# tgale96/sputnik

Hardware: AMD Instinct MI355X
Metric: effective TFLOP/s (nnz-FLOPs) DSD block=128 M=K=N=4096 @ 1/2/4/8 GPU vs density (higher is better)
Workload: dtype f16

## Files before the change

### sputnik_amd/csrc/api_internal.h

```cpp
#ifndef SPUTNIK_AMD_API_INTERNAL_H_
#define SPUTNIK_AMD_API_INTERNAL_H_

#include <cstddef>

#include "sputnik/block/arguments.h"

namespace sputnik_amd {

enum class Status {
  kOk,
  kNotSupported,
  kNoKernel,
  kMissingMetadata,
  kMissingRowIndices,
};

using sputnik::block::BlockMatrix;
using sputnik::block::Matrix;

struct Workspace {
  void *ptr = nullptr;
  size_t bytes = 0;
};

// ... 76 lines not shown
void SetPairFault(int on);
int CaptureWorkspaces();
int SelectDsdKernel(int four_wave);
bool Dsd4wEnabled();
bool Dsd4wForced();
int Dsd4wEpi();

enum KnobId {
  kKnobPairs,
  kKnobPairXcd2,
  kKnobSplit,
  kKnobSplitMinBn,
  kKnobDsd4w,
  kKnobGroupedSdd,
  kKnobGroupedMinPerCu,
  kKnobTall,
  kKnobTallPersistent,
  kKnobDdsXcd2,
  kKnobSdd4wMaxLd,
  kKnobPairFault,
  kKnobSddKsplit,
  kKnobSddKsplitMinK,
  kKnobSddOrder,
  kKnobTall4w,
  kKnobTallFlushW,
  kKnobTallOddShare,
  kKnobMinHandoff,
  kKnobXcdRows,
  kKnobSddKrot,
  kKnobSddSpread,
  kKnobSddBtMinMib,
  kKnobSddTailMinK,
  kKnobSddActRoute,
  kNumKnobs
};
int Knob(KnobId k);
int TuningGet(const char *name);
int TuningSet(const char *name, int value);

}

#endif
```

### sputnik_amd/csrc/block_gemm.h

```cpp
#ifndef SPUTNIK_AMD_BLOCK_GEMM_H_
#define SPUTNIK_AMD_BLOCK_GEMM_H_

#include <hip/hip_runtime.h>
#include <stdint.h>

#include <type_traits>

#include "act_math.h"

#ifndef SPUTNIK_EXP
#define SPUTNIK_EXP 0
#endif
#ifndef SPUTNIK_S_AUX
#define SPUTNIK_S_AUX 0
#endif
#ifndef SPUTNIK_D_AUX
#define SPUTNIK_D_AUX 0
#endif
#ifndef SPUTNIK_IDX_PREFETCH
#define SPUTNIK_IDX_PREFETCH 0
#endif
#ifndef SPUTNIK_READ_FIRST
#define SPUTNIK_READ_FIRST 0
#endif
// ... 56 lines not shown
  int grid;
  int persistent;
  unsigned long long *tile_counter;
  int pair;
  float *pair_partials;
  unsigned *pair_flags;
  unsigned pair_epoch;
  unsigned *pair_sync;
  unsigned *pair_error;
  int pair_fault;
  int pair_xcd2;
  int pair_split;
  int split_bn;
  unsigned long long *debug;
  const int *d_offsets;
  const short *d_indices;
  const int *d_block_offsets;
  int s_blocks;
  int sdd_ksplit;
  unsigned *ks_flags;
  int sdd_order;
  int tall_flush_w;
  int tall_odd_share;
  int min_handoff;
  int xcd_rows;
  int sdd_krot;
  int sdd_spread;
  int sdd_tail;
  int tail_cus;
  char *z_data;
  int act;
  char *u_data;
  char *du_data;
};

__device__ __forceinline__ int tr_key(int k) {
  return (k & 3) | (((k >> 3) & 1) << 2);
}
template <int kChunks>
__device__ __forceinline__ int kc_key(int row) {
  return (row >> 1) & (kChunks - 1);
}

template <typename T>
struct MfmaTraits;
template <>
struct MfmaTraits<_Float16> {
  static __device__ __forceinline__ f32x4 mfma(s16x8 a, s16x8 b, f32x4 c) {
    return __builtin_amdgcn_mfma_f32_16x16x32_f16(
        __builtin_bit_cast(f16x8, a), __builtin_bit_cast(f16x8, b), c, 0, 0,
        0);
  }
};
template <>
struct MfmaTraits<__bf16> {
  static __device__ __forceinline__ f32x4 mfma(s16x8 a, s16x8 b, f32x4 c) {
    return __builtin_amdgcn_mfma_f32_16x16x32_bf16(
        __builtin_bit_cast(bf16x8, a), __builtin_bit_cast(bf16x8, b), c, 0, 0,
        0);
  }
};

template <int N>
__device__ __forceinline__ void wait_vmcnt() {
  asm volatile("s_waitcnt vmcnt(%0)" ::"n"(N) : "memory");
}
// ... 1618 lines not shown
```

### sputnik_amd/csrc/dispatch.cpp

```cpp
#include <atomic>
#include <cstdint>
#include <cstdlib>
#include <cstring>
#include <mutex>

#include "api_internal.h"
#include "block_gemm.h"
#include "dsd4w.h"
#include "layout.h"
#include "metadata.h"
#include "sputnik/sputnik.h"
#include "sputnik_amd.h"

namespace sputnik_amd {

static unsigned long long *g_debug = nullptr;

constexpr int kMaxDevices = 64;

static std::atomic<unsigned long long> g_incall_events{0};
static std::atomic<unsigned long long> g_bt_launches{0};
static thread_local int t_product_depth = 0;
struct InProduct {
  InProduct() { ++t_product_depth; }
// ... 37 lines not shown
static std::mutex g_pairs_mu;

struct KnobDef {
  const char *name;
  const char *env;
  int def, lo, hi;
};
static const KnobDef kKnobs[kNumKnobs] = {
    {"pairs", "SPUTNIK_AMD_PAIRS", 1, 0, 1},
    {"pair_xcd2", "SPUTNIK_AMD_PAIR_XCD2", 3, 0, 3},
    {"split", "SPUTNIK_AMD_SPLIT", 1, 0, 1},
    {"split_min_bn", "SPUTNIK_AMD_SPLIT_MIN_BN", 128, 0, 1 << 20},
    {"dsd4w", "SPUTNIK_AMD_DSD4W", 1, 0, 7},
    {"grouped_sdd", "SPUTNIK_AMD_GROUPED_SDD", 1, 0, 1},
    {"grouped_min_per_cu", "SPUTNIK_AMD_GROUPED_MIN_PER_CU", 4, 0, 1 << 20},
    {"tall", "SPUTNIK_AMD_TALL", 1, 0, 2},
    {"tall_persistent", "SPUTNIK_AMD_TALL_PERSISTENT", 1, 0, 1},
    {"dds_xcd2", "SPUTNIK_AMD_DDS_XCD2", 3, 0, 3},
    {"sdd4w_max_ld", "SPUTNIK_AMD_SDD4W_MAX_LD", 16384, 0, 1 << 30},
    {"pair_fault", "SPUTNIK_AMD_PAIR_FAULT", 0, 0, 1},
    {"sdd_ksplit", "SPUTNIK_AMD_SDD_KSPLIT", 1, 1, 8},
    {"sdd_ksplit_min_k", "SPUTNIK_AMD_SDD_KSPLIT_MIN_K", 6144, 512, 1 << 30},
    {"sdd_order", "SPUTNIK_AMD_SDD_ORDER", 1, 0, 4},
    {"tall4w", "SPUTNIK_AMD_TALL4W", 1, 0, 1},
    {"tall_flush_w", "SPUTNIK_AMD_TALL_FLUSH_W", 4, 0, 64},
    {"tall_odd_share", "SPUTNIK_AMD_TALL_ODD_SHARE", 120, 50, 200},
    {"min_handoff", "SPUTNIK_AMD_MIN_HANDOFF", 2, 1, 64},
    {"xcd_rows", "SPUTNIK_AMD_XCD_ROWS", 1, 0, 1},
    {"sdd_krot", "SPUTNIK_AMD_SDD_KROT", 0, 0, 4},
    {"sdd_spread", "SPUTNIK_AMD_SDD_SPREAD", 2, 0, 2},
    {"sdd_bt_min_mib", "SPUTNIK_AMD_SDD_BT_MIN_MIB", 256, 0, 1 << 20},
    {"sdd_tail_min_k", "SPUTNIK_AMD_SDD_TAIL_MIN_K", 8192, 0, 1 << 30},
    {"sdd_act_route", "SPUTNIK_AMD_SDD_ACT_ROUTE", 0, 0, 2},
};
constexpr int kKnobUnset = -0x7fffffff - 1;
static std::atomic<int> g_knobs[kNumKnobs];
static std::once_flag g_knobs_once;

static void InitKnobs() {
  std::call_once(g_knobs_once, [] {
    for (int i = 0; i < kNumKnobs; ++i) {
      const char *e = std::getenv(kKnobs[i].env);
      char *end = nullptr;
      const long v0 = e != nullptr && *e != 0 ? std::strtol(e, &end, 10) : 0;
      const bool ok = e != nullptr && *e != 0 && end != nullptr && *end == 0 &&
                      v0 >= kKnobs[i].lo && v0 <= kKnobs[i].hi;
      const int v = ok ? (int)v0 : kKnobs[i].def;
      g_knobs[i].store(v, std::memory_order_relaxed);
    }
  });
}

int Knob(KnobId k) {
  InitKnobs();
  return g_knobs[k].load(std::memory_order_relaxed);
}

static int KnobIndex(const char *name) {
  if (name == nullptr) return -1;
  for (int i = 0; i < kNumKnobs; ++i)
    if (std::strcmp(name, kKnobs[i].name) == 0) return i;
  return -1;
}

int TuningGet(const char *name) {
  const int i = KnobIndex(name);
// ... 1021 lines not shown
        return RunDsd(a, ta, Matrix(b.cols, b.rows, bt), false, c, dtype, build_meta, stream,
                      st_out, Workspace{}, OutMode::kStore);
      }
    }
  }
  if (needs_meta && build_meta) {
    const hipError_t e = BuildTransposed(a, stream);
    if (e != hipSuccess) return e;
  }
  p.debug = g_debug;
  p.xcd_rows = Knob(kKnobXcdRows);
  PreparePairs(&p, a.nonzeros / (kBlock * kBlock), stream);
  const GemmParams p0 = p;
  GemmParams pd = p;
  const bool tall = UseTall(&pd, stream, true);
  if (tall && UseTallPipe(p0, a.nonzeros / (kBlock * kBlock),
                          ((long long)a.cols + kBlock - 1) / kBlock, ta, tb)) {
    GemmParams q = p0;
    q.persistent = 0;
    q.num_jtiles = q.j_limit / 512;
    q.tall_flush_w = Knob(kKnobTallFlushW);
    q.tall_odd_share = Knob(kKnobTallOddShare);
    int dev = 0;
    q.num_tiles = hipGetDevice(&dev) == hipSuccess ? DeviceCUs(dev) : 0;
    return LaunchDsd4w(dtype, q, 7, false, stream, false, false);
  }
  if (tall) (void)UseTall(&p, stream);
  if (Dsd4wEnabled() &&
      Dsd4wApplies(p, Dsd4wForced() ? (1LL << 40) : a.nonzeros / (kBlock * kBlock),
                   !ta, tb, false, tall)) {
    int epi = Dsd4wEpi();
    if (Dsd4wMode() == 1 && a.nonzeros / (kBlock * kBlock) < 12LL * p.num_rows)
      epi = 5;
    return LaunchDsd4w(dtype, p, epi, tb && !ta, stream, ta && !tb, ta && tb);
  }
  return LaunchBlockGemm(dtype, false, !ta, tb, false, tall, p, stream);
}

hipError_t RunDds(const Matrix &a, bool ta, const BlockMatrix &b, bool tb,
                  const Matrix &c, int dtype, bool build_meta,
                  hipStream_t stream, Status *st_out, OutMode out) {
  const InProduct in_product;
  GemmParams p;
  bool needs_meta = false;
  const Status st = PrepareDds(a, ta, b, tb, c, &p, &needs_meta);
  *st_out = st;
  if (st != Status::kOk) return hipSuccess;
  if (needs_meta && build_meta) {
    const hipError_t e = BuildTransposed(b, stream);
    if (e != hipSuccess) return e;
  }
  p.debug = g_debug;
  if (out != OutMode::kStore) {
    if (out == OutMode::kAccF32) p.c_ld *= 2;
    PreparePairs(&p, b.nonzeros / (kBlock * kBlock), stream, false,
                 false);
    const bool tall = UseTall(&p, stream);
    return LaunchBlockGemmAcc(dtype, tb, !ta,
                              true, tall,
                              out == OutMode::kAccF32 ? kOutAccF32 : kOutAccT,
                              p, stream);
  }
  p.xcd_rows = Knob(kKnobXcdRows);
  PreparePairs(&p, b.nonzeros / (kBlock * kBlock), stream);
  const bool tall = UseTall(&p, stream);
  if (Dsd4wEnabled() &&
// ... 707 lines not shown
```

### sputnik_amd/csrc/dsd4w.hip

```cpp
#include <hip/hip_runtime.h>
#include <stdint.h>

#include <cstdlib>

#include "api_internal.h"
#include "block_gemm.h"
#include "dsd4w.h"
#include "dsd4w_asm.inc"

namespace sputnik_amd {
namespace {

constexpr int kRankScratch = 24576;
constexpr uint32_t kOob = 0x80000000u;

struct Pick {
  int row_a, row_b, e_a, n_a, e_b, n_b, target;
  int uniform;
};

__device__ Pick rank_wave(const GemmParams &p, char *lds, int wave, int lane,
                          int ra, int rb, int o0_pre, bool pre) {
  const int R = p.num_rows;
  const int o0 = pre ? o0_pre : lane <= R ? p.s_offsets[lane] : 0;
// ... 78 lines not shown
  out.n_b = __builtin_amdgcn_readfirstlane(offs[out.row_b + 1]) - out.e_b;
  __syncthreads();
  return out;
}

__device__ __forceinline__ unsigned long long exp_stamp(int dep) {
#if (SPUTNIK_EXP & 512) != 0
  unsigned long long t;
  asm volatile("s_memrealtime %0\n s_waitcnt lgkmcnt(0)"
               : "=s"(t) : "s"(__builtin_amdgcn_readfirstlane(dep)));
  return t;
#else
  (void)dep;
  return 0;
#endif
}

template <bool kBf16, int kEpi, bool kDds, bool kSdd = false, bool kNt = false,
          bool kTt = false, bool kTn = false>
__global__ void __launch_bounds__(256, 1) dsd4w_kernel(const GemmParams p) {
  constexpr bool kWaveEpi = kEpi != 0;
  constexpr bool kDs = kEpi == 3 || kEpi == 4 || kEpi == 5 || kEpi == 6 || kEpi == 7;
  constexpr bool kBar2 = kEpi == 4;
  constexpr bool kKs = kEpi == 6;
  constexpr bool kTp = kEpi == 7;
  static_assert(!kTp || (!kSdd && !kDds && !kNt && !kTt && !kTn), "tall pipeline: DSD NN");
  static_assert(!kDds || kEpi == 1 || kEpi == 3, "DDS: per-wave epilogue only");
  static_assert(!kSdd || ((kEpi == 3 || (kEpi == 4 && !kTt) || (kEpi == 1 && kTn) ||
                           (kKs && !kNt && !kTt && !kTn)) && !kDds),
                "SDD: double slots (TN: per-step images), per-wave epilogue");
  static_assert(!kKs || kSdd, "K-split: SDD NN only");
  constexpr bool kARowsT = (kTt || kTn) && kSdd;
  constexpr bool kDdsTt = kDds && kTt;
  [[maybe_unused]] const unsigned long long t_entry = __builtin_amdgcn_s_memrealtime();
  __shared__ __attribute__((aligned(1024))) char lds[163840];
  const int tid = threadIdx.x;
  const int lane = tid & 63;
  const int wave = __builtin_amdgcn_readfirstlane(tid >> 6);
  const uint32_t lbase =
      (uint32_t)(uintptr_t)((__attribute__((address_space(3))) char *)lds);

  constexpr int kIdxPreload = 1024;
  const int nb_all = p.s_blocks;
  [[maybe_unused]] const unsigned long long t_karg = exp_stamp(nb_all);
  const bool idx_pre = nb_all <= kIdxPreload &&
                       (reinterpret_cast<uintptr_t>(p.s_indices) & 15) == 0;
  typedef unsigned v4u_t __attribute__((ext_vector_type(4)));
  v4u_t idx_lo = {0u, 0u, 0u, 0u}, idx_hi = {0u, 0u, 0u, 0u};
  if (idx_pre) {
    const __amdgpu_buffer_rsrc_t ri = __builtin_amdgcn_make_buffer_rsrc(
        const_cast<short *>(p.s_indices), 0, (nb_all * 2 + 3) & ~3, 0x00020000);
    idx_lo = __builtin_bit_cast(v4u_t, __builtin_amdgcn_raw_buffer_load_b128(
                                            ri, lane * 32, 0, 0));
    idx_hi = __builtin_bit_cast(v4u_t, __builtin_amdgcn_raw_buffer_load_b128(
                                            ri, lane * 32 + 16, 0, 0));
  }
#ifndef SPUTNIK_OFF_EARLY
#define SPUTNIK_OFF_EARLY 1
#endif
  const bool off_early = SPUTNIK_OFF_EARLY && !kSdd && !kTp && p.num_rows < 64;
  int off_pre = 0;
  if (off_early && lane <= p.num_rows) off_pre = p.s_offsets[lane];
  auto kblock_of = [&](int e) {
    if constexpr (kSdd) return e;
    if (!idx_pre || e >= nb_all) return scalar_load_short(p.s_indices, e);
    const int l = e >> 4, d = (e & 15) >> 1;
    const unsigned w0 = __builtin_amdgcn_readlane(idx_lo.x, l);
    const unsigned w1 = __builtin_amdgcn_readlane(idx_lo.y, l);
    const unsigned w2 = __builtin_amdgcn_readlane(idx_lo.z, l);
    const unsigned w3 = __builtin_amdgcn_readlane(idx_lo.w, l);
    const unsigned w4 = __builtin_amdgcn_readlane(idx_hi.x, l);
    const unsigned w5 = __builtin_amdgcn_readlane(idx_hi.y, l);
    const unsigned w6 = __builtin_amdgcn_readlane(idx_hi.z, l);
    const unsigned w7 = __builtin_amdgcn_readlane(idx_hi.w, l);
    const unsigned w = d == 0 ? w0 : d == 1 ? w1 : d == 2 ? w2 : d == 3 ? w3
                     : d == 4 ? w4 : d == 5 ? w5 : d == 6 ? w6 : w7;
    return (int)((e & 1) ? (w >> 16) : (w & 0xffff));
  };

  int srow, j0;
  int b1, n1, b2 = 0, n2 = 0;
  bool producer = false, collect = false;
  int pair_id = 0;
  [[maybe_unused]] unsigned long long t_rank = 0;
  unsigned epoch = p.pair_epoch;
  if (p.pair != 0 && p.pair_sync != nullptr)
    epoch = ((unsigned)scalar_load_int(reinterpret_cast<const int *>(p.pair_sync), 0) &
             0x7fffffffu) + 1u;
  int grp_b0 = 0, grp_count = 0, grp_c = 0;
  bool split_idle = false;
  int kss = 1, kch = 0, kofs = 0;
  unsigned tp_ent = 0, tp_tile = 0, tp_ent2 = 0, tp_tile2 = 0, tp_zero = 0xffffffffu;
  int tp_first = 0, tp_second = 0, tp_nzero = 0;
  if constexpr (kSdd) {
    int tile = xcd_tile(blockIdx.x, gridDim.x);
    const int R = !kKs && p.sdd_tail != 0
                      ? sdd_tail_rows<256>(p, reinterpret_cast<int *>(lds + kRankScratch), tid)
                      : p.num_rows;
    const bool band = p.sdd_order >= 1;
    const int per = band ? ((R + 255) / 256 + 7) & ~7 : (R + 255) / 256;
    const int r0 = min(R, tid * per), r1 = min(R, r0 + per);
    int local = 0, gmin = 0x7fffffff, gmax = 0;
    for (int r = r0; r < r1; ++r) {
      const int gr = (p.c_offsets[r + 1] - p.c_offsets[r] + 3) / 4;
      local += gr;
      gmin = min(gmin, gr);
      gmax = max(gmax, gr);
    }
    int incl = local;
#pragma unroll
    for (int d = 1; d < 64; d <<= 1) {
      const int v = __shfl_up(incl, d, 64);
      if (lane >= d) incl += v;
    }
#pragma unroll
    for (int d = 1; d < 64; d <<= 1) {
      gmin = min(gmin, __shfl_xor(gmin, d, 64));
      gmax = max(gmax, __shfl_xor(gmax, d, 64));
    }
    int *wsum = reinterpret_cast<int *>(lds + kRankScratch);
    if (lane == 63) {
      wsum[wave] = incl;
      wsum[4 + wave] = gmin;
      wsum[8 + wave] = gmax;
// ... 224 lines not shown
      }
      __syncthreads();
      tp_nzero = min(64, zhi - zlo);
      tp_zero = lane < tp_nzero ? (unsigned)zl[lane] : 0xffffffffu;
    }
    __syncthreads();
    j0 = 0;
    srow = 0;
    b1 = 0;
    n1 = nblk;
    tp_first = (int)(__builtin_amdgcn_readlane(tp_ent, 0) & 0xffffffu);
    tp_second = (int)(__builtin_amdgcn_readlane(tp_ent, nblk > 1 ? 1 : 0) & 0xffffffu);
    split_idle = nblk == 0;
  } else if (p.pair != 0 && p.pair_split == 2) {
    const int nt = p.num_tiles;
    const int gch = (int)blockIdx.x >= nt ? 1 : 0;
    const int t = xcd_tile((int)blockIdx.x - gch * nt, nt);
    srow = t % p.num_rows;
    j0 = (t / p.num_rows) * 512;
    const int e_r = scalar_load_int(p.s_offsets, srow);
    const int n_r = scalar_load_int(p.s_offsets, srow + 1) - e_r;
    const int c0 = gch * n_r / 2, c1 = (gch + 1) * n_r / 2;
    b1 = e_r + c0;
    n1 = c1 - c0;
    pair_id = t;
    if (gch == 0) {
      producer = n1 > 0;
      split_idle = n1 == 0;
    } else {
      collect = n_r / 2 > 0;
    }
  } else if (p.pair != 0) {
    const int R = p.num_rows;
    const int half = R >> 1;
    const int n_light = p.num_jtiles * half;
    const int n_solo = p.num_jtiles * (R & 1);
    const int bid = blockIdx.x;
    int role, panel, pi;
    const bool xcd2 = p.pair_xcd2 != 0 && p.num_jtiles == 8 && n_solo == 0 &&
                      (half & 1) == 0;
    const int rot = xcd2 ? xcd_rotation() : 0;
    auto place = [&](int b) {
      if (xcd2) {
        const int x = b & 7, k = b >> 3;
        panel = 2 * (x >> 1) + (k & 1);
        pi = p.pair_xcd2 == 2 ? 2 * (k >> 1) + (x & 1)
           : (fast_xcd(x, rot) ^ (p.pair_xcd2 == 3 ? 1 : 0)) * (half >> 1) + (k >> 1);
      } else {
        const int t = xcd_tile(b, n_light);
        panel = t / half;
        pi = t % half;
      }
    };
    if (bid < n_light) {
      role = 0;
      place(bid);
    } else if (bid < n_light + n_solo) {
      role = 1;
      panel = bid - n_light;
      pi = half;
    } else {
      role = 2;
      place(bid - n_light - n_solo);
    }
    const Pick rp = R < 64 ? rank_wave(p, lds, wave, lane, pi, R - 1 - pi, off_pre, off_early)
                           : rank_block(p, lds, tid, pi, R - 1 - pi);
    t_rank = exp_stamp(rp.target + rp.e_a + rp.e_b);
    const int min_handoff = p.min_handoff > 0 ? p.min_handoff : SPUTNIK_MIN_HANDOFF;
    int hb = role == 1 ? 0 : rp.n_a - rp.target;
    if (hb < min_handoff) hb = 0;
    pair_id = panel * half + pi;
    j0 = panel * 512;
    if (role == 0) {
      srow = rp.row_b;
      b1 = rp.e_a;
      n1 = hb;
      b2 = rp.e_b;
      n2 = rp.n_b;
      producer = hb > 0;
    } else {
      srow = rp.row_a;
      b1 = rp.e_a + hb;
      n1 = rp.n_a - hb;
      collect = hb > 0;
    }
  } else {
    const int tile = xcd_tile(blockIdx.x, gridDim.x);
    const int panel = tile / p.num_rows;
    const int target = tile % p.num_rows;
    j0 = panel * 512;
    if (p.num_rows < 64) {
      const Pick rp = rank_wave(p, lds, wave, lane, target, target, off_pre, off_early);
      srow = rp.row_a;
      b1 = rp.e_a;
      n1 = rp.n_a;
    } else if (p.num_rows <= kLptRows) {
      const Pick rp = rank_block(p, lds, tid, target, target);
      srow = rp.row_a;
      b1 = rp.e_a;
      n1 = rp.n_a;
      const int R = p.num_rows;
      if (p.xcd_rows != 0 && rp.uniform != 0 && (R & 7) == 0 &&
          (int)gridDim.x == p.num_tiles) {
        const int rx = R >> 3, x = (int)blockIdx.x & 7, tx = (int)blockIdx.x >> 3;
        srow = x * rx + tx % rx;
        j0 = (tx / rx) * 512;
        const int *offs = reinterpret_cast<const int *>(lds + kRankScratch);
        b1 = __builtin_amdgcn_readfirstlane(offs[srow]);
      }
    } else {
      srow = target;
      b1 = scalar_load_int(p.s_offsets, srow);
      n1 = scalar_load_int(p.s_offsets, srow + 1) - b1;
    }
  }
  srow = __builtin_amdgcn_readfirstlane(srow);
  j0 = __builtin_amdgcn_readfirstlane(j0);
  const int ntot = n1 + n2;

  typedef unsigned v4u __attribute__((ext_vector_type(4)));
  if (split_idle) {
  } else if (ntot == 0 && kDds) {
    const v4u z = {0u, 0u, 0u, 0u};
    for (int id = tid; id < 512 * 16; id += 256) {
      const int r = id >> 4, cc = id & 15;
      if (j0 + r >= p.j_limit) continue;
      __builtin_nontemporal_store(
          z, reinterpret_cast<v4u *>(p.c_data + (long long)(j0 + r) * p.c_ld +
                                     (long long)srow * 256 + cc * 16));
    }
  } else if (ntot == 0) {
    const v4u z = {0u, 0u, 0u, 0u};
    for (int id = tid; id < 128 * 64; id += 256) {
      const int r = id >> 6, cc = id & 63;
      const int jc = j0 + cc * 8;
      if (jc >= p.j_limit) continue;
      __builtin_nontemporal_store(
          z, reinterpret_cast<v4u *>(p.c_data + ((long long)srow * 128 + r) * p.c_ld +
                                     (long long)jc * 2));
    }
  } else {
    const int b2m = b2 - n1;
    const int xlast = ntot - 1;
    auto entry = [&](int x) { return x + (x < n1 ? b1 : b2m); };
    const int kb0 = kblock_of(kTp ? tp_first : entry(0));
    const int kb1 = kblock_of(kTp ? tp_second : entry(xlast < 1 ? xlast : 1));
    constexpr bool kColOrder =
        !kDdsTt && ((kDds && !kNt) || ((kTn || kTt) && !kSdd));
    const int bo0 = kColOrder ? scalar_load_int(p.s_block_offsets, entry(0)) : 0;
    const int bo1 =
        kColOrder ? scalar_load_int(p.s_block_offsets, entry(xlast < 1 ? xlast : 1)) : 0;
    [[maybe_unused]] const unsigned long long t_kb = exp_stamp(kb0 + kb1);

    uint32_t vs, vs1 = 0;
    if constexpr (!kDdsTt && ((kDds && !kNt) || kTt || kTn)) {
      const int k = 8 * wave + (lane >> 4);
      const int pc = lane & 15;
      const int c = (((pc >> 1) ^ tr_key(k)) << 1) | (pc & 1);
      vs = (uint32_t)(k * (kARowsT ? p.s_ld : 256) + c * 16);
    } else if constexpr (kDs) {
      const long long srs = kSdd ? p.s_ld : 256;
      auto off = [&](int x) {
        const int r = 32 * wave + 8 * x + (lane >> 3);
        return (uint32_t)(r * srs + (((lane & 7) ^ ((r >> 1) & 7)) << 4));
      };
      vs = off(0);
      vs1 = off(1);
    } else {
      const int srow_l = 32 * wave + (lane >> 2);
      vs = (uint32_t)(srow_l * 256 + (((lane & 3) ^ ((srow_l >> 1) & 3)) << 4));
    }
    uint32_t vd[2];
#pragma unroll
    for (int x = 0; x < 2; ++x) {
      if constexpr (!kDdsTt && ((kDds && kDs) || kNt || kTt)) {
        const int r = 8 * x + (lane >> 3);
        vd[x] = j0 + 128 * wave < p.j_limit
                    ? (uint32_t)(r * p.d_ld + (((lane & 7) ^ ((r >> 1) & 7)) << 4))
                    : kOob;
      } else if constexpr (kDds && !kTn && !kDdsTt) {
        const int r = lane >> 2;
        vd[x] = j0 + 128 * wave < p.j_limit
                    ? (uint32_t)(r * p.d_ld + (((lane & 3) ^ ((r >> 1) & 3)) << 4))
                    : kOob;
      } else {
        const int k = (lane >> 4) + 8 * x;
        const int pc = lane & 15;
        const int c = (((pc >> 1) ^ tr_key(k)) << 1) | (pc & 1);
        const int col = (kSdd ? grp_c * 128 : j0 + 128 * wave) + c * 8;
        vd[x] = col < p.j_limit ? (uint32_t)((lane >> 4) * p.d_ld + c * 16) : kOob;
      }
    }
    const uint32_t own = lbase + 32768u + 32768u * wave;
    const int r16 = lane & 15, g = lane >> 4;
    const uint32_t vrs =
        (kDds ? own : lbase) +
        (kDs ? (uint32_t)(r16 * 128 + ((g ^ ((r16 >> 1) & 7)) << 4))
             : (uint32_t)(r16 * 64 + ((g ^ ((r16 >> 1) & 3)) << 4)));
    const uint32_t vrs1 = vrs ^ 64u;
    const int q = (lane >> 2) & 3, pp = lane & 3;
    const int kr = 8 * g + q;
    uint32_t vrd[8];
#pragma unroll
    for (int n = 0; n < 8; ++n)
      vrd[n] = (kDds || kTt ? lbase : own) +
               (uint32_t)(kr * 256 + pp * 8 + ((n ^ tr_key(kr)) << 5));
    uint32_t vrt[8];
#pragma unroll
    for (int m = 0; m < 8; ++m)
      vrt[m] = (kDds ? own : lbase) +
               (uint32_t)(kr * 256 + pp * 8 + ((m ^ tr_key(kr)) << 5));
    const uint32_t vrk0 = (kDds ? lbase : own) +
                          (uint32_t)(r16 * 128 + ((g ^ ((r16 >> 1) & 7)) << 4));
    const uint32_t vrk1 = vrk0 ^ 64u;
    const uint32_t vw0 = lbase + (uint32_t)(r16 * 1040 + (128 * wave + 4 * g) * 2);
    const uint32_t vw1 = vw0 + 64 * 1040;
    const uint32_t wreg = lbase + 32768u + 32768u * wave;
    uint32_t vws[8], vrb[4];
#pragma unroll
    for (int n = 0; n < 8; ++n)
      vws[n] = wreg + (uint32_t)(r16 * 256 + (((2 * n + (g >> 1)) ^ r16) << 4) + 8 * (g & 1));
#pragma unroll
    for (int qq = 0; qq < 4; ++qq) {
      const int rr = 4 * qq + g;
      vrb[qq] = wreg + (uint32_t)(rr * 256 + ((r16 ^ rr) << 4));
    }
    const bool cvalid = kSdd   ? wave < grp_count
                        : kDds ? j0 + 128 * wave < p.j_limit
                               : j0 + 128 * wave + r16 * 8 < p.j_limit;
    const long long cld = kSdd ? 256 : p.c_ld;
    const uint32_t vco = cvalid ? (uint32_t)(g * cld + r16 * 16) : kOob;
    const uint32_t vpl = (uint32_t)(wave * 65536 + lane * 16);
    const uint32_t vcl = (uint32_t)((lane & 15) * p.c_ld + (lane >> 4) * 8);

    auto U = [](uint32_t x) { return (uint32_t)__builtin_amdgcn_readfirstlane((int)x); };
    auto U64 = [&](uint64_t x) {
      return (uint64_t)U((uint32_t)x) | ((uint64_t)U((uint32_t)(x >> 32)) << 32);
    };
    const uint64_t sd = U64((uint64_t)(
        p.s_data + (kARowsT ? (long long)srow * 256
                    : kSdd  ? (long long)srow * 128 * p.s_ld + (long long)kofs * 256 : 0)));
    const uint64_t dt = U64((uint64_t)(
        p.d_data + (kDdsTt ? (long long)(j0 + 128 * wave) * 2
                    : (kNt || kTt) && !kSdd ? (long long)(j0 + 128 * wave) * p.d_ld
                    : kNt || kTt ? (long long)grp_c * 128 * p.d_ld
                    : kSdd ? (long long)grp_c * 256 + (long long)kofs * 128 * p.d_ld
                           : (long long)(j0 + 128 * wave) * (kDds && !kTn ? p.d_ld : 2))));
    const uint64_t ix = U64((uint64_t)p.s_indices);
    const uint64_t pd =
        U64((uint64_t)(p.pair_partials + (long long)pair_id * 128 * 512));
    const uint64_t flag_p =
        U64(kKs ? (uint64_t)(p.ks_flags + pair_id)
            : p.pair != 0 ? (uint64_t)(p.pair_flags + pair_id) : 0);
    const uint64_t err_p = U64((uint64_t)p.pair_error);
    constexpr bool kKcD = !kDdsTt && ((kDds && !kTn) || kNt || kTt);
    const uint32_t k128 = U((uint32_t)(kKcD ? 256 : 128 * p.d_ld));
    const uint32_t k32 = U((uint32_t)(kKcD ? 64 : 32 * p.d_ld));
    const uint32_t k4 = U((uint32_t)(kKcD ? 16 * p.d_ld : 4 * p.d_ld));
    const uint32_t ms =
        U(lbase + ((kDs && (((!kDds || kNt) && !kTt) || kDdsTt)) ? 4096u : 2048u) * wave);
    const uint32_t sk32 = U((uint32_t)(kARowsT ? 32 * p.s_ld : 0));
    const uint32_t sk128 = U((uint32_t)(kARowsT ? 128 * p.s_ld : 0));
    const uint32_t md = U(lbase + 32768u + 32768u * wave);
    const uint32_t flushrem = U(producer ? (uint32_t)n2 : 0xffffffffu);
    const uint32_t pubat = U(producer && n2 > 0 ? (uint32_t)n2 + 1u : 0u);
    const uint32_t publast = U(producer && n2 == 0 ? 1u : 0u);
    const bool clb = collect && ntot >= 3;
    const uint32_t clbf = U(clb ? 2u : 0xffffffffu), clbc = U(clb ? 1u : 0xffffffffu);
    const bool split_first = p.pair != 0 && p.pair_split == 2 && producer;
    const uint32_t flags =
        U((collect ? 1u : 0u) | (!collect && !(producer && n2 == 0) ? 2u : 0u) |
          (p.pair_fault ? 4u : 0u) | (wave == 3 ? 8u : 0u) | (wave == 0 ? 16u : 0u) |
          (split_first ? 32u : 0u) | (kKs && wave >= grp_count ? 64u : 0u));
    const uint64_t cd = U64(
        kSdd ? (uint64_t)(p.c_data + (long long)(grp_b0 + wave) * 32768)
        : kDds ? (uint64_t)(p.c_data + (long long)(j0 + 128 * wave) * p.c_ld +
                          (long long)srow * 256)
             : (uint64_t)(p.c_data + (long long)srow * 128 * p.c_ld +
                          (long long)(j0 + 128 * wave) * 2));
    const uint64_t bo = U64((uint64_t)p.s_block_offsets);
    const uint32_t c4 = U((uint32_t)(4 * cld));
    const uint32_t s16 = U((uint32_t)(kARowsT ? 4 * p.s_ld : kSdd ? 16 * p.s_ld : 0));
    const uint32_t ub1 = U(b1), un1 = U(n1), ub2m = U(b2m), uxlast = U(xlast),
                   untot = U(ntot), ukb0 = U(kb0), ukb1 = U(kb1), uep = U(epoch),
                   ubo0 = U(bo0), ubo1 = U(bo1), ukss = U(kss), ukch = U(kch);
    const uint32_t crow = U((uint32_t)(128 * p.c_ld));
    const uint32_t unz = U((uint32_t)tp_nzero);

#define DSD4W_INPUTS                                                           \
    [sdlo] "s"((uint32_t)sd), [sdhi] "s"((uint32_t)(sd >> 32)),               \
    [dtlo] "s"((uint32_t)dt), [dthi] "s"((uint32_t)(dt >> 32)),               \
    [k128] "s"(k128), [k32] "s"(k32), [k4] "s"(k4),                            \
    [ixlo] "s"((uint32_t)ix), [ixhi] "s"((uint32_t)(ix >> 32)),               \
    [b1] "s"(ub1), [n1] "s"(un1), [b2m] "s"(ub2m), [xlast] "s"(uxlast),        \
    [ntot] "s"(untot), [kb0] "s"(ukb0), [kb1] "s"(ukb1),                       \
    [flushrem] "s"(flushrem),                                                  \
    [pdlo] "s"((uint32_t)pd), [pdhi] "s"((uint32_t)(pd >> 32)),               \
    [flag] "s"(flag_p), [epoch] "s"(uep), [flags] "s"(flags),                  \
    [err] "s"(err_p), [ms] "s"(ms),                                            \
    [md] "s"(md), [vs] "v"(vs), [vd0] "v"(vd[0]), [vd1] "v"(vd[1]),           \
    [vrs] "v"(vrs), [vrd0] "v"(vrd[0]), [vrd1] "v"(vrd[1]),                   \
    [vs1] "v"(vs1), [vrs1] "v"(vrs1), [s16] "s"(s16),                          \
    [vrk0] "v"(vrk0), [vrk1] "v"(vrk1), [sk32] "s"(sk32), [sk128] "s"(sk128),  \
    [vrt0] "v"(vrt[0]), [vrt1] "v"(vrt[1]), [vrt2] "v"(vrt[2]), [vrt3] "v"(vrt[3]), \
    [vrt4] "v"(vrt[4]), [vrt5] "v"(vrt[5]), [vrt6] "v"(vrt[6]), [vrt7] "v"(vrt[7]), \
    [vrd2] "v"(vrd[2]), [vrd3] "v"(vrd[3]), [vrd4] "v"(vrd[4]),               \
    [vrd5] "v"(vrd[5]), [vrd6] "v"(vrd[6]), [vrd7] "v"(vrd[7]),               \
    [vpl] "v"(vpl), [bolo] "s"((uint32_t)bo), [bohi] "s"((uint32_t)(bo >> 32)),  \
    [bo0] "s"(ubo0), [bo1] "s"(ubo1), [pubat] "s"(pubat), [clbf] "s"(clbf),  \
    [clbc] "s"(clbc), [publast] "s"(publast), [kss] "s"(ukss), [kch] "s"(ukch), \
    [vent] "v"(tp_ent), [vtile] "v"(tp_tile), [vent2] "v"(tp_ent2),         \
    [vtile2] "v"(tp_tile2), [vcl] "v"(vcl), [crow] "s"(crow),                \
    [vzero] "v"(tp_zero), [nzero] "s"(unz)
#define DSD4W_OPERANDS : DSD4W_INPUTS
#define DSD4W_OPERANDS_G DSD4W_OPERANDS, [vw0] "v"(vw0), [vw1] "v"(vw1)
#define DSD4W_INPUTS_W                                                         \
  DSD4W_INPUTS, [cdlo] "s"((uint32_t)cd), [cdhi] "s"((uint32_t)(cd >> 32)),  \
      [c4] "s"(c4), [vws0] "v"(vws[0]), [vws1] "v"(vws[1]), [vws2] "v"(vws[2]), \
      [vws3] "v"(vws[3]), [vws4] "v"(vws[4]), [vws5] "v"(vws[5]),               \
      [vws6] "v"(vws[6]), [vws7] "v"(vws[7]), [vrb0] "v"(vrb[0]),               \
// ... 422 lines not shown
```

Before: 1156.

## Prefetch dense operand rows and hoist tile placement before row ranking in DSD 4-wave

Moves the pair/tile placement computation ahead of the rank step so each block knows its column panel early. The blocks then issue a spread of buffer loads covering the first few K-block rows of the dense B operand, warming cache while the ranking and metadata loads run. It also touches the kernarg cache lines up front and gates the entry timestamp behind an experiment flag. An optional early lane-setup path exists but is off by default. The warm loads cost extra VGPRs and memory traffic, which may hurt occupancy or compete with the main loads.

```diff
diff --git a/sputnik_amd/csrc/api_internal.h b/sputnik_amd/csrc/api_internal.h
--- a/sputnik_amd/csrc/api_internal.h
+++ b/sputnik_amd/csrc/api_internal.h
@@ -132,6 +132,7 @@
   kKnobSddBtMinMib,
   kKnobSddTailMinK,
   kKnobSddActRoute,
+  kKnobDWarm,
   kNumKnobs
 };
 int Knob(KnobId k);
diff --git a/sputnik_amd/csrc/block_gemm.h b/sputnik_amd/csrc/block_gemm.h
--- a/sputnik_amd/csrc/block_gemm.h
+++ b/sputnik_amd/csrc/block_gemm.h
@@ -112,6 +112,8 @@
   int act;
   char *u_data;
   char *du_data;
+  int d_warm;
+  long long d_bytes;
 };
 
 __device__ __forceinline__ int tr_key(int k) {
diff --git a/sputnik_amd/csrc/dispatch.cpp b/sputnik_amd/csrc/dispatch.cpp
--- a/sputnik_amd/csrc/dispatch.cpp
+++ b/sputnik_amd/csrc/dispatch.cpp
@@ -93,6 +93,7 @@
     {"sdd_bt_min_mib", "SPUTNIK_AMD_SDD_BT_MIN_MIB", 256, 0, 1 << 20},
     {"sdd_tail_min_k", "SPUTNIK_AMD_SDD_TAIL_MIN_K", 8192, 0, 1 << 30},
     {"sdd_act_route", "SPUTNIK_AMD_SDD_ACT_ROUTE", 0, 0, 2},
+    {"d_warm", "SPUTNIK_AMD_D_WARM", 1, 0, 2},
 };
 constexpr int kKnobUnset = -0x7fffffff - 1;
 static std::atomic<int> g_knobs[kNumKnobs];
@@ -1180,6 +1181,16 @@
     int epi = Dsd4wEpi();
     if (Dsd4wMode() == 1 && a.nonzeros / (kBlock * kBlock) < 12LL * p.num_rows)
       epi = 5;
+    const int warm = Knob(kKnobDWarm);
+    const long long blocks = a.nonzeros / (kBlock * kBlock);
+    const long long kblocks = ((long long)a.cols + kBlock - 1) / kBlock;
+    const long long b_bytes = (((long long)b.rows - 1) * (p.d_ld / 2) + b.cols) * 2;
+    if (warm != 0 && !ta && !tb && !tall && p.num_rows < 64 &&
+        (warm == 2 || blocks >= 8LL * p.num_rows) && b.rows > 0 && b_bytes > 0 &&
+        b_bytes <= (long long)kNumRecords) {
+      p.d_warm = (int)std::min(4LL, kblocks);
+      p.d_bytes = b_bytes;
+    }
     return LaunchDsd4w(dtype, p, epi, tb && !ta, stream, ta && !tb, ta && tb);
   }
   return LaunchBlockGemm(dtype, false, !ta, tb, false, tall, p, stream);
diff --git a/sputnik_amd/csrc/dsd4w.hip b/sputnik_amd/csrc/dsd4w.hip
--- a/sputnik_amd/csrc/dsd4w.hip
+++ b/sputnik_amd/csrc/dsd4w.hip
@@ -134,7 +134,16 @@
   static_assert(!kKs || kSdd, "K-split: SDD NN only");
   constexpr bool kARowsT = (kTt || kTn) && kSdd;
   constexpr bool kDdsTt = kDds && kTt;
-  [[maybe_unused]] const unsigned long long t_entry = __builtin_amdgcn_s_memrealtime();
+  [[maybe_unused]] const unsigned long long t_entry =
+      (SPUTNIK_EXP & 512) != 0 ? __builtin_amdgcn_s_memrealtime() : 0ull;
+  {
+    const __attribute__((address_space(4))) int *ka =
+        (const __attribute__((address_space(4))) int *)__builtin_amdgcn_kernarg_segment_ptr();
+    constexpr int kLast = (int)sizeof(GemmParams) / 4 - 1;
+    static_assert(sizeof(GemmParams) > 320 && sizeof(GemmParams) <= 384, "kernarg lines");
+    asm volatile("" ::"s"(ka[0]), "s"(ka[16]), "s"(ka[32]), "s"(ka[48]), "s"(ka[64]),
+                 "s"(ka[80]), "s"(ka[kLast]));
+  }
   __shared__ __attribute__((aligned(1024))) char lds[163840];
   const int tid = threadIdx.x;
   const int lane = tid & 63;
@@ -192,6 +201,240 @@
   int grp_b0 = 0, grp_count = 0, grp_c = 0;
   bool split_idle = false;
   int kss = 1, kch = 0, kofs = 0;
+
+  constexpr bool kEarly = !kSdd && !kTp;
+#ifndef SPUTNIK_SETUP_EARLY
+#define SPUTNIK_SETUP_EARLY 0
+#endif
+  constexpr bool kLanesEarly = kEarly && SPUTNIK_SETUP_EARLY != 0;
+  const bool one_tile = kEarly && !(p.pair != 0 && p.pair_split == 2);
+  int role = 0, panel = 0, pi = 0;
+  int warm_s = 0, warm_ns = 0;
+  if (one_tile && p.pair != 0) {
+    const int R = p.num_rows;
+    const int half = R >> 1;
+    const int n_light = p.num_jtiles * half;
+    const int n_solo = p.num_jtiles * (R & 1);
+    const int bid = blockIdx.x;
+    const bool xcd2 = p.pair_xcd2 != 0 && p.num_jtiles == 8 && n_solo == 0 &&
+                      (half & 1) == 0;
+    const int rot = xcd2 ? xcd_rotation() : 0;
+    auto place = [&](int b, int second) {
+      if (xcd2) {
+        const int x = b & 7, k = b >> 3;
+        panel = 2 * (x >> 1) + (k & 1);
+        pi = p.pair_xcd2 == 2 ? 2 * (k >> 1) + (x & 1)
+           : (fast_xcd(x, rot) ^ (p.pair_xcd2 == 3 ? 1 : 0)) * (half >> 1) + (k >> 1);
+        warm_s = (k >> 1) + second * (half >> 1);
+        warm_ns = half;
+      } else {
+        const int t = xcd_tile(b, n_light);
+        panel = t / half;
+        pi = t % half;
+        warm_s = pi + second * half;
+        warm_ns = 2 * half;
+      }
+    };
+    if (bid < n_light) {
+      role = 0;
+      place(bid, 0);
+    } else if (bid < n_light + n_solo) {
+      role = 1;
+      panel = bid - n_light;
+      pi = half;
+    } else {
+      role = 2;
+      place(bid - n_light - n_solo, 1);
+    }
+    pair_id = panel * half + pi;
+  } else if (one_tile) {
+    const int tile = xcd_tile(blockIdx.x, gridDim.x);
+    panel = tile / p.num_rows;
+    pi = tile % p.num_rows;
+    warm_s = pi;
+    warm_ns = p.num_rows;
+  }
+  const int j0_early = __builtin_amdgcn_readfirstlane(panel * 512);
+  const int pair_id_early = pair_id;
+
+  constexpr bool kWarm = kEarly && !kDds && !kNt && !kTt && !kTn;
+  constexpr int kWarmLoads = 8;
+  v4u_t warm[kWarmLoads];
+#pragma unroll
+  for (int i = 0; i < kWarmLoads; ++i) warm[i] = v4u_t{0u, 0u, 0u, 0u};
+  if constexpr (kWarm) {
+    const bool warm_on = one_tile && p.d_warm > 0 && warm_ns > 0;
+    const long long bytes = warm_on ? p.d_bytes : 0;
+    uint32_t wo[kWarmLoads];
+#pragma unroll
+    for (int i = 0; i < kWarmLoads; ++i) wo[i] = kOob;
+    if (warm_on) {
+      const int chunks = p.d_warm * 128 * 64;
+      const int per = (int)(((unsigned)chunks + (unsigned)warm_ns - 1u) / (unsigned)warm_ns);
+      const int c0 = warm_s * per, c1 = min(chunks, c0 + per);
+      const int c = c0 + tid;
+      const int col = j0_early + (c & 63) * 8;
+      const long long o0 = (long long)(c >> 6) * p.d_ld + (long long)col * 2;
+#pragma unroll
+      for (int i = 0; i < kWarmLoads; ++i) {
+        const long long o = o0 + (long long)(4 * i) * p.d_ld;
+        const bool ok = c + 256 * i < c1 && col < p.j_limit && o + 16 <= bytes;
+        wo[i] = ok ? (uint32_t)o : kOob;
+      }
+    }
+    const __amdgpu_buffer_rsrc_t rw = __builtin_amdgcn_make_buffer_rsrc(
+        const_cast<char *>(p.d_data), 0, (int)bytes, 0x00020000);
+#pragma unroll
+    for (int i = 0; i < kWarmLoads; ++i)
+      warm[i] = __builtin_bit_cast(
+          v4u_t, __builtin_amdgcn_raw_buffer_load_b128(rw, wo[i], 0, 0));
+  }
+
+  auto U = [](uint32_t x) { return (uint32_t)__builtin_amdgcn_readfirstlane((int)x); };
+  auto U64 = [&](uint64_t x) {
+    return (uint64_t)U((uint32_t)x) | ((uint64_t)U((uint32_t)(x >> 32)) << 32);
+  };
+  struct LaneSetup {
+    uint32_t vs, vs1, vrs, vrs1, vrd[8], vrt[8], vrk0, vrk1, vw0, vw1, vws[8], vrb[4],
+        vpl, vcl;
+    uint64_t ix, err_p, bo;
+    uint32_t k128, k32, k4, ms, sk32, sk128, md, c4, s16, crow;
+  };
+  struct TileSetup {
+    uint32_t vd[2], vco;
+    uint64_t sd, dt, pd, flag_p;
+  };
+  auto lane_setup = [&]() {
+    LaneSetup o;
+    o.vs1 = 0;
+    if constexpr (!kDdsTt && ((kDds && !kNt) || kTt || kTn)) {
+      const int k = 8 * wave + (lane >> 4);
+      const int pc = lane & 15;
+      const int c = (((pc >> 1) ^ tr_key(k)) << 1) | (pc & 1);
+      o.vs = (uint32_t)(k * (kARowsT ? p.s_ld : 256) + c * 16);
+    } else if constexpr (kDs) {
+      const long long srs = kSdd ? p.s_ld : 256;
+      auto off = [&](int x) {
+        const int r = 32 * wave + 8 * x + (lane >> 3);
+        return (uint32_t)(r * srs + (((lane & 7) ^ ((r >> 1) & 7)) << 4));
+      };
+      o.vs = off(0);
+      o.vs1 = off(1);
+    } else {
+      const int srow_l = 32 * wave + (lane >> 2);
+      o.vs = (uint32_t)(srow_l * 256 + (((lane & 3) ^ ((srow_l >> 1) & 3)) << 4));
+    }
+    const uint32_t own = lbase + 32768u + 32768u * wave;
+    const int r16 = lane & 15, g = lane >> 4;
+    o.vrs = (kDds ? own : lbase) +
+            (kDs ? (uint32_t)(r16 * 128 + ((g ^ ((r16 >> 1) & 7)) << 4))
+                 : (uint32_t)(r16 * 64 + ((g ^ ((r16 >> 1) & 3)) << 4)));
+    o.vrs1 = o.vrs ^ 64u;
+    const int q = (lane >> 2) & 3, pp = lane & 3;
+    const int kr = 8 * g + q;
+#pragma unroll
+    for (int n = 0; n < 8; ++n)
+      o.vrd[n] = (kDds || kTt ? lbase : own) +
+                 (uint32_t)(kr * 256 + pp * 8 + ((n ^ tr_key(kr)) << 5));
+#pragma unroll
+    for (int m = 0; m < 8; ++m)
+      o.vrt[m] = (kDds ? own : lbase) +
+                 (uint32_t)(kr * 256 + pp * 8 + ((m ^ tr_key(kr)) << 5));
+    o.vrk0 = (kDds ? lbase : own) +
+             (uint32_t)(r16 * 128 + ((g ^ ((r16 >> 1) & 7)) << 4));
+    o.vrk1 = o.vrk0 ^ 64u;
+    o.vw0 = lbase + (uint32_t)(r16 * 1040 + (128 * wave + 4 * g) * 2);
+    o.vw1 = o.vw0 + 64 * 1040;
+    const uint32_t wreg = lbase + 32768u + 32768u * wave;
+#pragma unroll
+    for (int n = 0; n < 8; ++n)
+      o.vws[n] = wreg + (uint32_t)(r16 * 256 + (((2 * n + (g >> 1)) ^ r16) << 4) + 8 * (g & 1));
+#pragma unroll
+    for (int qq = 0; qq < 4; ++qq) {
+      const int rr = 4 * qq + g;
+      o.vrb[qq] = wreg + (uint32_t)(rr * 256 + ((r16 ^ rr) << 4));
+    }
+    o.vpl = (uint32_t)(wave * 65536 + lane * 16);
+    o.vcl = (uint32_t)((lane & 15) * p.c_ld + (lane >> 4) * 8);
+    o.ix = U64((uint64_t)p.s_indices);
+    o.err_p = U64((uint64_t)p.pair_error);
+    constexpr bool kKcD = !kDdsTt && ((kDds && !kTn) || kNt || kTt);
+    o.k128 = U((uint32_t)(kKcD ? 256 : 128 * p.d_ld));
+    o.k32 = U((uint32_t)(kKcD ? 64 : 32 * p.d_ld));
+    o.k4 = U((uint32_t)(kKcD ? 16 * p.d_ld : 4 * p.d_ld));
+    o.ms =
+        U(lbase + ((kDs && (((!kDds || kNt) && !kTt) || kDdsTt)) ? 4096u : 2048u) * wave);
+    o.sk32 = U((uint32_t)(kARowsT ? 32 * p.s_ld : 0));
+    o.sk128 = U((uint32_t)(kARowsT ? 128 * p.s_ld : 0));
+    o.md = U(lbase + 32768u + 32768u * wave);
+    o.bo = U64((uint64_t)p.s_block_offsets);
+    const long long cld = kSdd ? 256 : p.c_ld;
+    o.c4 = U((uint32_t)(4 * cld));
+    o.s16 = U((uint32_t)(kARowsT ? 4 * p.s_ld : kSdd ? 16 * p.s_ld : 0));
+    o.crow = U((uint32_t)(128 * p.c_ld));
+    return o;
+  };
+  auto tile_setup = [&](int j0v, int slot, int srow_v) {
+    TileSetup o;
+#pragma unroll
+    for (int x = 0; x < 2; ++x) {
+      if constexpr (!kDdsTt && ((kDds && kDs) || kNt || kTt)) {
+        const int r = 8 * x + (lane >> 3);
+        o.vd[x] = j0v + 128 * wave < p.j_limit
+                      ? (uint32_t)(r * p.d_ld + (((lane & 7) ^ ((r >> 1) & 7)) << 4))
+                      : kOob;
+      } else if constexpr (kDds && !kTn && !kDdsTt) {
+        const int r = lane >> 2;
+        o.vd[x] = j0v + 128 * wave < p.j_limit
+                      ? (uint32_t)(r * p.d_ld + (((lane & 3) ^ ((r >> 1) & 3)) << 4))
+                      : kOob;
+      } else {
+        const int k = (lane >> 4) + 8 * x;
+        const int pc = lane & 15;
+        const int c = (((pc >> 1) ^ tr_key(k)) << 1) | (pc & 1);
+        const int col = (kSdd ? grp_c * 128 : j0v + 128 * wave) + c * 8;
+        o.vd[x] = col < p.j_limit ? (uint32_t)((lane >> 4) * p.d_ld + c * 16) : kOob;
+      }
+    }
+    const int r16 = lane & 15, g = lane >> 4;
+    const bool cvalid = kSdd   ? wave < grp_count
+                        : kDds ? j0v + 128 * wave < p.j_limit
+                               : j0v + 128 * wave + r16 * 8 < p.j_limit;
+    const long long cld = kSdd ? 256 : p.c_ld;
+    o.vco = cvalid ? (uint32_t)(g * cld + r16 * 16) : kOob;
+    o.sd = U64((uint64_t)(
+        p.s_data + (kARowsT ? (long long)srow_v * 256
+                    : kSdd  ? (long long)srow_v * 128 * p.s_ld + (long long)kofs * 256 : 0)));
+    o.dt = U64((uint64_t)(
+        p.d_data + (kDdsTt ? (long long)(j0v + 128 * wave) * 2
+                    : (kNt || kTt) && !kSdd ? (long long)(j0v + 128 * wave) * p.d_ld
+                    : kNt || kTt ? (long long)grp_c * 128 * p.d_ld
+                    : kSdd ? (long long)grp_c * 256 + (long long)kofs * 128 * p.d_ld
+                           : (long long)(j0v + 128 * wave) * (kDds && !kTn ? p.d_ld : 2))));
+    o.pd = U64((uint64_t)(p.pair_partials + (long long)slot * 128 * 512));
+    o.flag_p = U64(kKs ? (uint64_t)(p.ks_flags + slot)
+                   : p.pair != 0 ? (uint64_t)(p.pair_flags + slot) : 0);
+    return o;
+  };
+  LaneSetup ls;
+  TileSetup ts;
+  if constexpr (kLanesEarly) {
+    ls = lane_setup();
+    ts = tile_setup(j0_early, pair_id_early, 0);
+    asm volatile(""
+                 : "+v"(ls.vs), "+v"(ls.vs1), "+v"(ls.vrs), "+v"(ls.vrs1), "+v"(ls.vrd[0]),
+                   "+v"(ls.vrd[1]), "+v"(ls.vrd[2]), "+v"(ls.vrd[3]), "+v"(ls.vrd[4]),
+                   "+v"(ls.vrd[5]), "+v"(ls.vrd[6]), "+v"(ls.vrd[7]), "+v"(ls.vrt[0]),
+                   "+v"(ls.vrt[1]), "+v"(ls.vrt[2]), "+v"(ls.vrt[3]), "+v"(ls.vrt[4]),
+                   "+v"(ls.vrt[5]), "+v"(ls.vrt[6]), "+v"(ls.vrt[7]), "+v"(ls.vrk0),
+                   "+v"(ls.vrk1), "+v"(ls.vw0), "+v"(ls.vw1), "+v"(ls.vpl), "+v"(ls.vcl));
+    asm volatile(""
+                 : "+v"(ls.vws[0]), "+v"(ls.vws[1]), "+v"(ls.vws[2]), "+v"(ls.vws[3]),
+                   "+v"(ls.vws[4]), "+v"(ls.vws[5]), "+v"(ls.vws[6]), "+v"(ls.vws[7]),
+                   "+v"(ls.vrb[0]), "+v"(ls.vrb[1]), "+v"(ls.vrb[2]), "+v"(ls.vrb[3]),
+                   "+v"(ts.vd[0]), "+v"(ts.vd[1]), "+v"(ts.vco));
+  }
+
   unsigned tp_ent = 0, tp_tile = 0, tp_ent2 = 0, tp_tile2 = 0, tp_zero = 0xffffffffu;
   int tp_first = 0, tp_second = 0, tp_nzero = 0;
   if constexpr (kSdd) {
@@ -482,45 +725,13 @@
     }
   } else if (p.pair != 0) {
     const int R = p.num_rows;
-    const int half = R >> 1;
-    const int n_light = p.num_jtiles * half;
-    const int n_solo = p.num_jtiles * (R & 1);
-    const int bid = blockIdx.x;
-    int role, panel, pi;
-    const bool xcd2 = p.pair_xcd2 != 0 && p.num_jtiles == 8 && n_solo == 0 &&
-                      (half & 1) == 0;
-    const int rot = xcd2 ? xcd_rotation() : 0;
-    auto place = [&](int b) {
-      if (xcd2) {
-        const int x = b & 7, k = b >> 3;
-        panel = 2 * (x >> 1) + (k & 1);
-        pi = p.pair_xcd2 == 2 ? 2 * (k >> 1) + (x & 1)
-           : (fast_xcd(x, rot) ^ (p.pair_xcd2 == 3 ? 1 : 0)) * (half >> 1) + (k >> 1);
-      } else {
-        const int t = xcd_tile(b, n_light);
-        panel = t / half;
-        pi = t % half;
-      }
-    };
-    if (bid < n_light) {
-      role = 0;
-      place(bid);
-    } else if (bid < n_light + n_solo) {
-      role = 1;
-      panel = bid - n_light;
-      pi = half;
-    } else {
-      role = 2;
-      place(bid - n_light - n_solo);
-    }
     const Pick rp = R < 64 ? rank_wave(p, lds, wave, lane, pi, R - 1 - pi, off_pre, off_early)
                            : rank_block(p, lds, tid, pi, R - 1 - pi);
     t_rank = exp_stamp(rp.target + rp.e_a + rp.e_b);
     const int min_handoff = p.min_handoff > 0 ? p.min_handoff : SPUTNIK_MIN_HANDOFF;
     int hb = role == 1 ? 0 : rp.n_a - rp.target;
     if (hb < min_handoff) hb = 0;
-    pair_id = panel * half + pi;
-    j0 = panel * 512;
+    j0 = j0_early;
     if (role == 0) {
       srow = rp.row_b;
       b1 = rp.e_a;
@@ -535,10 +746,8 @@
       collect = hb > 0;
     }
   } else {
-    const int tile = xcd_tile(blockIdx.x, gridDim.x);
-    const int panel = tile / p.num_rows;
-    const int target = tile % p.num_rows;
-    j0 = panel * 512;
+    const int target = pi;
+    j0 = j0_early;
     if (p.num_rows < 64) {
       const Pick rp = rank_wave(p, lds, wave, lane, target, target, off_pre, off_early);
       srow = rp.row_a;
@@ -602,116 +811,21 @@
         kColOrder ? scalar_load_int(p.s_block_offsets, entry(xlast < 1 ? xlast : 1)) : 0;
     [[maybe_unused]] const unsigned long long t_kb = exp_stamp(kb0 + kb1);
 
-    uint32_t vs, vs1 = 0;
-    if constexpr (!kDdsTt && ((kDds && !kNt) || kTt || kTn)) {
-      const int k = 8 * wave + (lane >> 4);
-      const int pc = lane & 15;
-      const int c = (((pc >> 1) ^ tr_key(k)) << 1) | (pc & 1);
-      vs = (uint32_t)(k * (kARowsT ? p.s_ld : 256) + c * 16);
-    } else if constexpr (kDs) {
-      const long long srs = kSdd ? p.s_ld : 256;
-      auto off = [&](int x) {
-        const int r = 32 * wave + 8 * x + (lane >> 3);
-        return (uint32_t)(r * srs + (((lane & 7) ^ ((r >> 1) & 7)) << 4));
-      };
-      vs = off(0);
-      vs1 = off(1);
-    } else {
-      const int srow_l = 32 * wave + (lane >> 2);
-      vs = (uint32_t)(srow_l * 256 + (((lane & 3) ^ ((srow_l >> 1) & 3)) << 4));
-    }
-    uint32_t vd[2];
-#pragma unroll
-    for (int x = 0; x < 2; ++x) {
-      if constexpr (!kDdsTt && ((kDds && kDs) || kNt || kTt)) {
-        const int r = 8 * x + (lane >> 3);
-        vd[x] = j0 + 128 * wave < p.j_limit
-                    ? (uint32_t)(r * p.d_ld + (((lane & 7) ^ ((r >> 1) & 7)) << 4))
-                    : kOob;
-      } else if constexpr (kDds && !kTn && !kDdsTt) {
-        const int r = lane >> 2;
-        vd[x] = j0 + 128 * wave < p.j_limit
-                    ? (uint32_t)(r * p.d_ld + (((lane & 3) ^ ((r >> 1) & 3)) << 4))
-                    : kOob;
-      } else {
-        const int k = (lane >> 4) + 8 * x;
-        const int pc = lane & 15;
-        const int c = (((pc >> 1) ^ tr_key(k)) << 1) | (pc & 1);
-        const int col = (kSdd ? grp_c * 128 : j0 + 128 * wave) + c * 8;
-        vd[x] = col < p.j_limit ? (uint32_t)((lane >> 4) * p.d_ld + c * 16) : kOob;
-      }
-    }
-    const uint32_t own = lbase + 32768u + 32768u * wave;
-    const int r16 = lane & 15, g = lane >> 4;
-    const uint32_t vrs =
-        (kDds ? own : lbase) +
-        (kDs ? (uint32_t)(r16 * 128 + ((g ^ ((r16 >> 1) & 7)) << 4))
-             : (uint32_t)(r16 * 64 + ((g ^ ((r16 >> 1) & 3)) << 4)));
-    const uint32_t vrs1 = vrs ^ 64u;
-    const int q = (lane >> 2) & 3, pp = lane & 3;
-    const int kr = 8 * g + q;
-    uint32_t vrd[8];
-#pragma unroll
-    for (int n = 0; n < 8; ++n)
-      vrd[n] = (kDds || kTt ? lbase : own) +
-               (uint32_t)(kr * 256 + pp * 8 + ((n ^ tr_key(kr)) << 5));
-    uint32_t vrt[8];
-#pragma unroll
-    for (int m = 0; m < 8; ++m)
-      vrt[m] = (kDds ? own : lbase) +
-               (uint32_t)(kr * 256 + pp * 8 + ((m ^ tr_key(kr)) << 5));
-    const uint32_t vrk0 = (kDds ? lbase : own) +
-                          (uint32_t)(r16 * 128 + ((g ^ ((r16 >> 1) & 7)) << 4));
-    const uint32_t vrk1 = vrk0 ^ 64u;
-    const uint32_t vw0 = lbase + (uint32_t)(r16 * 1040 + (128 * wave + 4 * g) * 2);
-    const uint32_t vw1 = vw0 + 64 * 1040;
-    const uint32_t wreg = lbase + 32768u + 32768u * wave;
-    uint32_t vws[8], vrb[4];
-#pragma unroll
-    for (int n = 0; n < 8; ++n)
-      vws[n] = wreg + (uint32_t)(r16 * 256 + (((2 * n + (g >> 1)) ^ r16) << 4) + 8 * (g & 1));
-#pragma unroll
-    for (int qq = 0; qq < 4; ++qq) {
-      const int rr = 4 * qq + g;
-      vrb[qq] = wreg + (uint32_t)(rr * 256 + ((r16 ^ rr) << 4));
-    }
-    const bool cvalid = kSdd   ? wave < grp_count
-                        : kDds ? j0 + 128 * wave < p.j_limit
-                               : j0 + 128 * wave + r16 * 8 < p.j_limit;
-    const long long cld = kSdd ? 256 : p.c_ld;
-    const uint32_t vco = cvalid ? (uint32_t)(g * cld + r16 * 16) : kOob;
-    const uint32_t vpl = (uint32_t)(wave * 65536 + lane * 16);
-    const uint32_t vcl = (uint32_t)((lane & 15) * p.c_ld + (lane >> 4) * 8);
-
-    auto U = [](uint32_t x) { return (uint32_t)__builtin_amdgcn_readfirstlane((int)x); };
-    auto U64 = [&](uint64_t x) {
-      return (uint64_t)U((uint32_t)x) | ((uint64_t)U((uint32_t)(x >> 32)) << 32);
-    };
-    const uint64_t sd = U64((uint64_t)(
-        p.s_data + (kARowsT ? (long long)srow * 256
-                    : kSdd  ? (long long)srow * 128 * p.s_ld + (long long)kofs * 256 : 0)));
-    const uint64_t dt = U64((uint64_t)(
-        p.d_data + (kDdsTt ? (long long)(j0 + 128 * wave) * 2
-                    : (kNt || kTt) && !kSdd ? (long long)(j0 + 128 * wave) * p.d_ld
-                    : kNt || kTt ? (long long)grp_c * 128 * p.d_ld
-                    : kSdd ? (long long)grp_c * 256 + (long long)kofs * 128 * p.d_ld
-                           : (long long)(j0 + 128 * wave) * (kDds && !kTn ? p.d_ld : 2))));
-    const uint64_t ix = U64((uint64_t)p.s_indices);
-    const uint64_t pd =
-        U64((uint64_t)(p.pair_partials + (long long)pair_id * 128 * 512));
-    const uint64_t flag_p =
-        U64(kKs ? (uint64_t)(p.ks_flags + pair_id)
-            : p.pair != 0 ? (uint64_t)(p.pair_flags + pair_id) : 0);
-    const uint64_t err_p = U64((uint64_t)p.pair_error);
-    constexpr bool kKcD = !kDdsTt && ((kDds && !kTn) || kNt || kTt);
-    const uint32_t k128 = U((uint32_t)(kKcD ? 256 : 128 * p.d_ld));
-    const uint32_t k32 = U((uint32_t)(kKcD ? 64 : 32 * p.d_ld));
-    const uint32_t k4 = U((uint32_t)(kKcD ? 16 * p.d_ld : 4 * p.d_ld));
-    const uint32_t ms =
-        U(lbase + ((kDs && (((!kDds || kNt) && !kTt) || kDdsTt)) ? 4096u : 2048u) * wave);
-    const uint32_t sk32 = U((uint32_t)(kARowsT ? 32 * p.s_ld : 0));
-    const uint32_t sk128 = U((uint32_t)(kARowsT ? 128 * p.s_ld : 0));
-    const uint32_t md = U(lbase + 32768u + 32768u * wave);
+    if constexpr (!kLanesEarly) {
+      ls = lane_setup();
+      ts = tile_setup(j0, pair_id, srow);
+    } else if (j0 != j0_early || pair_id != pair_id_early) {
+      ts = tile_setup(j0, pair_id, srow);
+    }
+    const uint32_t vs = ls.vs, vs1 = ls.vs1, vrs = ls.vrs, vrs1 = ls.vrs1;
+    const uint32_t *vd = ts.vd, *vrd = ls.vrd, *vrt = ls.vrt, *vws = ls.vws, *vrb = ls.vrb;
+    const uint32_t vrk0 = ls.vrk0, vrk1 = ls.vrk1, vpl = ls.vpl, vcl = ls.vcl;
+    [[maybe_unused]] const uint32_t vw0 = ls.vw0, vw1 = ls.vw1;
+    const uint32_t vco = ts.vco;
+    const uint64_t sd = ts.sd, dt = ts.dt, pd = ts.pd, flag_p = ts.flag_p;
+    const uint64_t ix = ls.ix, err_p = ls.err_p, bo = ls.bo;
+    const uint32_t k128 = ls.k128, k32 = ls.k32, k4 = ls.k4, ms = ls.ms, sk32 = ls.sk32,
+                   sk128 = ls.sk128, md = ls.md, c4 = ls.c4, s16 = ls.s16, crow = ls.crow;
     const uint32_t flushrem = U(producer ? (uint32_t)n2 : 0xffffffffu);
     const uint32_t pubat = U(producer && n2 > 0 ? (uint32_t)n2 + 1u : 0u);
     const uint32_t publast = U(producer && n2 == 0 ? 1u : 0u);
@@ -728,14 +842,13 @@
                           (long long)srow * 256)
              : (uint64_t)(p.c_data + (long long)srow * 128 * p.c_ld +
                           (long long)(j0 + 128 * wave) * 2));
-    const uint64_t bo = U64((uint64_t)p.s_block_offsets);
-    const uint32_t c4 = U((uint32_t)(4 * cld));
-    const uint32_t s16 = U((uint32_t)(kARowsT ? 4 * p.s_ld : kSdd ? 16 * p.s_ld : 0));
     const uint32_t ub1 = U(b1), un1 = U(n1), ub2m = U(b2m), uxlast = U(xlast),
                    untot = U(ntot), ukb0 = U(kb0), ukb1 = U(kb1), uep = U(epoch),
                    ubo0 = U(bo0), ubo1 = U(bo1), ukss = U(kss), ukch = U(kch);
-    const uint32_t crow = U((uint32_t)(128 * p.c_ld));
     const uint32_t unz = U((uint32_t)tp_nzero);
+    if constexpr (kWarm)
+      asm volatile("" ::"v"(warm[0]), "v"(warm[1]), "v"(warm[2]), "v"(warm[3]), "v"(warm[4]),
+                   "v"(warm[5]), "v"(warm[6]), "v"(warm[7]));
 
 #define DSD4W_INPUTS                                                           \
     [sdlo] "s"((uint32_t)sd), [sdhi] "s"((uint32_t)(sd >> 32)),               \
```

Result: no change. 1152 (-0.3%).
